# cvg/nice-slam

Hardware: NVIDIA H100
Metric: rendered rays/sec (higher is better)
Workload: dtype f32

## Files before the change

### nice_slam_b200/csrc/nsb_common.cuh

```cuda
#pragma once
#include <cuda_runtime.h>
#include <cuda_fp16.h>
#include <stdint.h>
#include "../../include/nice_slam_b200.h"

namespace nsb {

constexpr int kHid = 32;
constexpr int kEmb = 93;
constexpr int kEmbPad = 96;
constexpr int kChunk = 16;
constexpr int kRowF = 16;
constexpr int kMaxPtsPerBlock = 384;
constexpr int kMaxRaysPerBlock = 24;

__host__ __device__ inline size_t align16(size_t x) { return (x + 15) & ~size_t(15); }

template <int LV>
struct Dec {
  static constexpr bool XYZ = LV != 0;
  static constexpr int CD = LV == 2 ? 64 : 32;
  static constexpr int NO = LV == 3 ? 4 : 1;
  static constexpr int FIRST = XYZ ? kEmb : 32;
  static constexpr int FIRSTP = XYZ ? kEmbPad : 32;
// ... 129 lines not shown
  int max_n;
};
struct PeerTail { PeerX px; const double* loss; double* out13; };
struct FusedSeeds {
  int kind;
  const void* gt_rgb;
  const float* gt_depth_loss;
  double w_color;
  int handle_dynamic, use_color;
  double* g_depth; float* g_rgb; double* loss;
  double* res;
  int* counter;
  PeerX px;
};
int render_forward_fused(const nsb_render_inputs* in, const nsb_forward_outputs* out, const FusedSeeds* fs, void* stream,
                         const nsb_sampling* smp = nullptr);
int render_backward_tail(const nsb_render_inputs* in, const nsb_backward_args* bw, const PeerTail* tail, void* stream, bool after_forward = false,
                         const nsb_sampling* smp = nullptr);
int make_peerx(const struct nsb_peers* p, PeerX* px);
int eval_points_mesh(const nsb_render_inputs* in, const double* points, const nsb_mesh_lattice* lat, int n_points, float* raw, float* z,
                     void* stream);

size_t det_voxel_workspace_bytes(long long n_points);
int det_voxel_reduce(const nsb_grid& g, const int32_t* slot_map, const float* xn, const float* dc, long long n_points, float* d_grid,
                     void* workspace, size_t workspace_bytes, cudaStream_t st);
int det_tile_sum(const float* part, int tiles, int n_floats, float* out, cudaStream_t st);

void set_error(const char* fmt, ...);
int check_cuda(cudaError_t e, const char* what);

}
```

### nice_slam_b200/csrc/nsb_iter.cu

```cuda
#include <cstring>
#include "nsb_common.cuh"

using namespace nsb;

static size_t backward_offset(int n_rays) { return 16 + align16(nsb_tracking_seeds_workspace(n_rays)); }
static size_t split_offset(int n_rays) { return backward_offset(n_rays) + align16(nsb_backward_workspace_bytes()); }
extern "C" size_t nsb_iteration_workspace_bytes(int n_rays) {
  return split_offset(n_rays) + align16(nsb_split_workspace_bytes(n_rays, NSB_MAX_SAMPLES));
}
struct IterWs { int* seeds_counter; void* seeds_scratch; void* backward; void* split; size_t split_bytes; };
static IterWs carve(const nsb_iteration_buffers* b, int n_rays) {
  char* w = static_cast<char*>(b->workspace);
  return {reinterpret_cast<int*>(w), w + 16, w + backward_offset(n_rays), w + split_offset(n_rays), b->workspace_bytes - split_offset(n_rays)};
}

static int check_buffers(const nsb_render_inputs* in, const nsb_iteration_buffers* b, const nsb_backward_args* g) {
  if (!in || !b || !g) { set_error("iteration: NULL argument"); return NSB_ERR_ARG; }
  if (!b->depth || !b->var || !b->rgb || !b->z_vals || !b->raw || !b->g_depth || !b->g_rgb || !b->loss || !b->depth_max || !b->workspace) {
    set_error("iteration: incomplete nsb_iteration_buffers"); return NSB_ERR_ARG; }
  if (b->workspace_bytes < nsb_iteration_workspace_bytes(in->n_rays)) {
    int det = 0; nsb_get_option("deterministic", &det);
    set_error(det ? "iteration: workspace smaller than nsb_iteration_workspace_bytes(%d) with option deterministic on (size it after setting the option)"
                  : "iteration: workspace too small", in->n_rays);
    return NSB_ERR_ARG;
  }
  return NSB_OK;
}

static int forward_part(const nsb_render_inputs* in, const nsb_iteration_buffers* b, const IterWs& ws, nsb_render_inputs* in2, const FusedSeeds* fs,
                        void* stream, bool keep_depth_max = false) {
  *in2 = *in;
  if (!(keep_depth_max && in->depth_max != nullptr)) {
    in2->depth_max = nullptr;
    if (in->gt_depth && in->gt_depth_batch == nullptr && in->n_rays > NSB_INLINE_MAX_RAYS) {
      const int rc = nsb_batch_max_depth(in->gt_depth, in->n_rays, b->depth_max, stream); if (rc) return rc;
      in2->depth_max = b->depth_max;
    }
  }
  nsb_forward_outputs fo = {b->depth, b->var, b->rgb, b->z_vals, b->raw, nullptr, b->masks, ws.split, ws.split_bytes, b->acts, b->acts_levels};
  return render_forward_fused(in2, &fo, fs, stream);
}

static FusedSeeds fused_seeds(const nsb_iteration_buffers* b, const IterWs& ws, int kind, const void* gt_rgb, const float* gt_depth_loss, double w_color,
                              int handle_dynamic, int use_color, const PeerX* px) {
  FusedSeeds fs; memset(&fs, 0, sizeof(fs));
  fs.kind = kind; fs.gt_rgb = gt_rgb; fs.gt_depth_loss = gt_depth_loss; fs.w_color = w_color; fs.handle_dynamic = handle_dynamic; fs.use_color = use_color;
  fs.g_depth = b->g_depth; fs.g_rgb = b->g_rgb; fs.loss = b->loss; fs.counter = ws.seeds_counter;
  if (kind == 1) fs.res = static_cast<double*>(ws.seeds_scratch);
  if (px != nullptr) fs.px = *px;
  return fs;
}

static int backward_part(const nsb_render_inputs* in2, const nsb_iteration_buffers* b, const IterWs& ws, const nsb_backward_args* g, void* stream,
                         const PeerTail* tail = nullptr, bool after_forward = false) {
  nsb_backward_args bw = *g;
  bw.z_vals = b->z_vals; bw.raw = b->raw; bw.g_depth = b->g_depth; bw.g_var = nullptr; bw.g_rgb = b->g_rgb; bw.masks = b->masks; bw.acts = b->acts; bw.acts_levels = b->acts_levels;
  bw.workspace = ws.backward; bw.split_workspace = ws.split; bw.split_workspace_bytes = ws.split_bytes;
  if (b->event_bwd_begin) cudaEventRecord((cudaEvent_t)b->event_bwd_begin, (cudaStream_t)stream);
  const int rc = render_backward_tail(in2, &bw, tail, stream, after_forward && !b->event_bwd_begin);
  if (b->event_bwd_end) cudaEventRecord((cudaEvent_t)b->event_bwd_end, (cudaStream_t)stream);
  return rc;
}

extern "C" int nsb_tracking_iteration(const nsb_render_inputs* in, const nsb_iteration_buffers* buf, const double* gt_rgb,
                                      double w_color, int handle_dynamic, int use_color, const nsb_backward_args* grads, void* stream) {
  int rc = check_buffers(in, buf, grads); if (rc) return rc;
  if (!in->gt_depth) { set_error("tracking iteration needs gt_depth"); return NSB_ERR_ARG; }
  nsb_render_inputs in2;
  const bool fuse = in->n_rays > 0 && in->n_rays <= 512;
  if (fuse && use_color && !gt_rgb) { set_error("tracking iteration: use_color without gt_rgb"); return NSB_ERR_ARG; }
  const IterWs ws = carve(buf, in->n_rays);
  const FusedSeeds fs = fused_seeds(buf, ws, 1, gt_rgb, nullptr, w_color, handle_dynamic, use_color, nullptr);
  if ((rc = forward_part(in, buf, ws, &in2, fuse ? &fs : nullptr, stream))) return rc;
  if (!fuse && (rc = nsb_tracking_seeds(buf->depth, buf->var, buf->rgb, in->gt_depth, gt_rgb, in->n_rays, w_color, handle_dynamic, use_color,
// ... 39 lines not shown
```

### nice_slam_b200/csrc/nsb_render.cu

```cuda
#include <cstdarg>
#include <cstdio>
#include <cstring>
#include "nsb_common.cuh"
#include "nsb_geom.cuh"
#include "nsb_mlp.cuh"
#include "nsb_seeds.cuh"

namespace nsb {

__device__ __forceinline__ bool grid_fast(const nsb_grid& g) { return g.stride_c == 1; }

__device__ __forceinline__ float4 grid_load4(const nsb_grid& g, long long off, int c0, bool fast) {
  if (fast) return ldg_f4(g.data + off + c0);
  return make_float4(__ldg(g.data + off + (long long)c0 * g.stride_c), __ldg(g.data + off + (long long)(c0 + 1) * g.stride_c),
                     __ldg(g.data + off + (long long)(c0 + 2) * g.stride_c), __ldg(g.data + off + (long long)(c0 + 3) * g.stride_c));
}

__device__ __forceinline__ void gather_chunk(const nsb_grid& g, float* __restrict__ act, int row0, const float xn[3], int lane) {
  const bool fast = grid_fast(g);
  const int q = lane & 7;
#pragma unroll 2
  for (int it = 0; it < 4; it++) {
    const int pt = it * 4 + (lane >> 3);
    float x[3];
// ... 101 lines not shown
  int accumulate_rays;
  int split;
  int* group_done;
  float4* fwd_parts;
  double* ray_parts;
  int* ray_cnt;
  float4* tile_parts;
  int tile_rays;
  int kind_major;
  FusedSeeds fs;
  PeerTail tail;
  int acts_mask;
  int wbytes;
  int max_pts, max_rays;
  nsb_sampling smp;
};

struct MeshPoints { nsb_mesh_lattice lat; int lattice; float* z; };
struct DetParams { float* dc[4]; float* xn[4]; float* wpart[4]; };
__device__ __forceinline__ double lattice_value(const nsb_mesh_lattice& L, int a, int i) {
  return i == L.n[a] - 1 ? L.stop[a] : __dadd_rn(__dmul_rn((double)i, L.step[a]), L.start[a]);
}
__device__ __forceinline__ void mesh_point_geom(const KParams& P, const MeshPoints& M, long long gp, PointGeom& G) {
  double pin[3];
  if (M.lattice) {
    const long long nyz = (long long)M.lat.n[1] * M.lat.n[2];
    const int ix = (int)(gp / nyz), iy = (int)((gp - ix * nyz) / M.lat.n[2]), iz = (int)(gp - ix * nyz - (long long)iy * M.lat.n[2]);
    pin[0] = lattice_value(M.lat, 0, ix); pin[1] = lattice_value(M.lat, 1, iy); pin[2] = lattice_value(M.lat, 2, iz);
  } else {
    pin[0] = P.points[3 * gp]; pin[1] = P.points[3 * gp + 1]; pin[2] = P.points[3 * gp + 2];
// ... 137 lines not shown
  float carry = 1.0f;
  for (int base = 0; base < S; base += 32) {
    const int s = base + lane;
    const bool v = s < S;
    const float al = v ? sigmoid_f(10.0f * rw[4 * s + 3]) : 0.0f;
    const float q = v ? (1.0f - al) + 1e-10f : 1.0f;
    const float incl = warp_incl_prod(q, lane);
    float excl = __shfl_up_sync(0xffffffffu, incl, 1);
    if (lane == 0) excl = 1.0f;
    const float T = carry * excl;
    if (v) { wq[s] = al * T; if (tq) tq[s] = T; }
    carry *= __shfl_sync(0xffffffffu, incl, 31);
  }
}

__device__ __forceinline__ void composite_ray_outputs(const KParams& P, int ray, const float* rw, const double* z, float* wq, int lane) {
  const int S = P.S;
  ray_weights(rw, S, lane, wq, nullptr);
  __syncwarp();
  float c0 = 0.f, c1 = 0.f, c2 = 0.f; double dsum = 0.0;
  for (int s = lane; s < S; s += 32) {
    const float w = wq[s];
    c0 = fmaf(w, rw[4 * s], c0); c1 = fmaf(w, rw[4 * s + 1], c1); c2 = fmaf(w, rw[4 * s + 2], c2);
    dsum += (double)w * z[s];
  }
  c0 = warp_sum(c0); c1 = warp_sum(c1); c2 = warp_sum(c2); dsum = warp_sum(dsum);
  double v = 0.0;
  for (int s = lane; s < S; s += 32) { const double t = z[s] - dsum; v += (double)wq[s] * t * t; }
  v = warp_sum(v);
  if (lane == 0) {
    P.fo.depth[ray] = dsum; P.fo.var[ray] = v;
    P.fo.rgb[3 * ray] = c0; P.fo.rgb[3 * ray + 1] = c1; P.fo.rgb[3 * ray + 2] = c2;
  }
}

template <typename F>
__device__ __forceinline__ void composite_ray_backward(const float* rw, const double* z, int S, double gD, double gV, const float g3[3],
                                                       float* wq, float* tq, int lane, F&& store) {
  ray_weights(rw, S, lane, wq, tq);
  __syncwarp();
  double Dm = 0.0;
  for (int s = lane; s < S; s += 32) Dm += (double)wq[s] * z[s];
  Dm = warp_sum(Dm);
  double swt = 0.0;
  for (int s = lane; s < S; s += 32) swt += (double)wq[s] * (z[s] - Dm);
  swt = warp_sum(swt);
  const double gDe = gD + gV * (-2.0 * swt);
  float carry = 0.0f;
  const int nblk = (S + 31) / 32;
  for (int b = nblk - 1; b >= 0; b--) {
    const int s = b * 32 + lane;
    const bool v = s < S;
    float gw = 0.0f, al = 0.0f, T = 0.0f, w = 0.0f;
    if (v) {
      al = sigmoid_f(10.0f * rw[4 * s + 3]); T = tq[s]; w = wq[s];
      const double t = z[s] - Dm;
      gw = (float)(gDe * z[s] + gV * t * t) + g3[0] * rw[4 * s] + g3[1] * rw[4 * s + 1] + g3[2] * rw[4 * s + 2];
    }
    const float incl = warp_incl_suffix_sum(gw * w, lane);
    float excl = __shfl_down_sync(0xffffffffu, incl, 1);
    if (lane == 31) excl = 0.0f;
    const float R = carry + excl;
    if (v) {
      const float qd = (1.0f - al) + 1e-10f;
      store(s, w, al, T * gw - R / qd);
    }
    carry += __shfl_sync(0xffffffffu, incl, 0);
  }
}

__device__ __forceinline__ void store_ray_grad(const KParams& P, int ray, int a, double so, double sd) {
  if (P.accumulate_rays) {
    if (P.bw.d_rays_o != nullptr) so += (double)P.bw.d_rays_o[3 * ray + a];
    if (P.bw.d_rays_d != nullptr) sd += (double)P.bw.d_rays_d[3 * ray + a];
  }
  if (P.bw.d_rays_o != nullptr) P.bw.d_rays_o[3 * ray + a] = (float)so;
  if (P.bw.d_rays_d != nullptr) P.bw.d_rays_d[3 * ray + a] = (float)sd;
}

__device__ __forceinline__ void issue_weights(const KParams& P, const Smem& sm, int lv) {
  fence_proxy_async();
  const uint32_t bytes = (uint32_t)packed_floats(lv) * 4u;
  mbar_expect_tx(sm.bar, bytes);
// ... 76 lines not shown
}
__device__ __forceinline__ void fwd_composite_store(const KParams& P, const Smem& sm, const BlockRange& b, int warp, int warps, int lane) {
  const int r0 = b.r0, nr = b.nr, Pb = b.Pb;
  if (P.points != nullptr) {
    for (int lp = threadIdx.x; lp < Pb; lp += blockDim.x) {
      const long long gp = (long long)blockIdx.x * P.rays_per_block + lp;
      float4 v = *reinterpret_cast<float4*>(sm.raw + 4 * lp);
      if (!sm.inb[lp]) v.w = 100.0f;
      *reinterpret_cast<float4*>(P.points_raw + 4 * gp) = v;
    }
    return;
  }
  for (int lp = threadIdx.x; lp < Pb; lp += blockDim.x) if (!sm.inb[lp]) sm.raw[4 * lp + 3] = 100.0f;
  __syncthreads();
  for (int r = warp; r < nr; r += warps)
    composite_ray_outputs(P, r0 + r, sm.raw + 4 * r * P.S, sm.zs + r * P.S, sm.wgt + r * P.S, lane);
  const long long g0 = (long long)r0 * P.S;
  if (P.fo.z_vals != nullptr) for (int lp = threadIdx.x; lp < Pb; lp += blockDim.x) P.fo.z_vals[g0 + lp] = sm.zs[lp];
  if (P.fo.raw != nullptr)
    for (int lp = threadIdx.x; lp < Pb; lp += blockDim.x)
      *reinterpret_cast<float4*>(P.fo.raw + 4 * (g0 + lp)) = *reinterpret_cast<float4*>(sm.raw + 4 * lp);
}

__device__ __forceinline__ void fused_seeds_tail(const KParams& P, int n_participants, unsigned char* scratch) {
  if (P.fs.kind == 0) return;
  __shared__ int s_seeds_last;
  if (!grid_last_arrival(P.fs.counter, n_participants, &s_seeds_last)) return;
  if (P.fs.kind == 1) {
    tracking_seeds_body(P.fo.depth, P.fo.var, P.fo.rgb, P.in.gt_depth, static_cast<const double*>(P.fs.gt_rgb), P.in.n_rays, P.fs.w_color,
                        P.fs.handle_dynamic, P.fs.use_color, nullptr, 0, P.fs.g_depth, P.fs.g_rgb, P.fs.loss, P.fs.res, P.fs.px, scratch);
    if (P.fs.px.world > 1 && P.in.depth_max == nullptr && P.in.gt_depth_batch == nullptr && threadIdx.x == 0) peer_advance(P.fs.px, 0);
// ... 536 lines not shown
}

static void fill_common(KParams& K, const nsb_render_inputs* in) {
  K.in = *in;
  K.has_gt = (in->gt_depth != nullptr && in->stage != NSB_STAGE_COARSE) ? 1 : 0;
  K.S = in->n_samples + (K.has_gt ? in->n_surface : 0);
  K.n_dec = stage_decoders(in->stage, K.dec);
  for (int i = 0; i < 3; i++) K.dec_pos[i] = i;
  K.accumulate_rays = 0;
  K.split = 1; K.group_done = nullptr; K.fwd_parts = nullptr; K.ray_parts = nullptr; K.ray_cnt = nullptr; K.tile_parts = nullptr; K.tile_rays = 0; K.kind_major = 0;
  memset(&K.fs, 0, sizeof(K.fs)); memset(&K.tail, 0, sizeof(K.tail));
  K.points = nullptr; K.points_raw = nullptr; K.n_points = 0;
  K.acts_mask = in->stage == NSB_STAGE_COLOR ? 1 << NSB_COLOR : 0;
  memset(&K.smp, 0, sizeof(K.smp));
  for (int l = 0; l < 4; l++) K.d_packed[l] = nullptr;
}

constexpr int kMaxDevices = 64;
static int g_sm_count[kMaxDevices] = {0};
static int current_device() { int dev = 0; cudaGetDevice(&dev); return dev >= 0 && dev < kMaxDevices ? dev : 0; }
static int sm_count() {
  const int dev = current_device();
  if (g_sm_count[dev] == 0) { cudaDeviceGetAttribute(&g_sm_count[dev], cudaDevAttrMultiProcessorCount, dev); if (g_sm_count[dev] <= 0) g_sm_count[dev] = 132; }
  return g_sm_count[dev];
}

constexpr size_t kSmemCap = 226u * 1024u;
constexpr int kMaxPtsTc = 256;
static void choose_config(KParams& K, bool bwd, int max_pts_cap, int* warps = nullptr, size_t* smem = nullptr) {
  const int sms = sm_count();
// ... 260 lines not shown
  K.smp = *smp;
  if (smp->z_vals != nullptr) {
    if (smp->S < 1) { set_error("nsb_sampling.S = %d with a given z_vals", smp->S); return NSB_ERR_ARG; }
    K.S = smp->S; K.smp.lindisp = 0; K.smp.t_rand = nullptr;
  }
  return NSB_OK;
}

extern "C" int nsb_render_forward(const nsb_render_inputs* in, const nsb_forward_outputs* out, void* stream) {
  return nsb_render_forward_sampled(in, nullptr, out, stream);
}
extern "C" int nsb_render_forward_sampled(const nsb_render_inputs* in, const nsb_sampling* sampling, const nsb_forward_outputs* out, void* stream) {
  return nsb::render_forward_fused(in, out, nullptr, stream, sampling);
}
int nsb::render_forward_fused(const nsb_render_inputs* in, const nsb_forward_outputs* out, const nsb::FusedSeeds* fs, void* stream,
                              const nsb_sampling* smp) {
  int rc = validate_inputs(in, true); if (rc) return rc;
  if (!out || !out->depth || !out->var || !out->rgb) { set_error("forward outputs missing"); return NSB_ERR_ARG; }
  if (in->n_rays == 0) return NSB_OK;
  KParams K; fill_common(K, in); K.fo = *out; memset(&K.bw, 0, sizeof(K.bw));
  if ((rc = apply_sampling(K, smp))) return rc;
  if ((rc = apply_acts_levels(K, out->acts_levels))) return rc;
  if (fs != nullptr) K.fs = *fs;
  const Family fam = kernel_family(K.S, in->n_rays, false);
  if (fam == Family::Fma) K.fo.masks = nullptr;
  if (K.S > NSB_MAX_SAMPLES) { set_error("n_samples+n_surface = %d exceeds %d", K.S, NSB_MAX_SAMPLES); return NSB_ERR_UNSUPPORTED; }
  if (K.has_gt && in->n_surface > 0 && !in->t_surface) { set_error("t_surface NULL"); return NSB_ERR_ARG; }
  if ((rc = set_attrs())) return rc;
  if (K.fs.px.world > 1 && !(fam != Family::Fma && in->gt_depth != nullptr)) {
    set_error("in-kernel exchanges of a sharded forward need a tensor-core back-end and <= %d rays per rank", NSB_INLINE_MAX_RAYS); return NSB_ERR_UNSUPPORTED; }
  if (fam == Family::Tile) {
    if (!out->z_vals || !out->raw) { set_error("the tensor-core forward needs z_vals and raw outputs"); return NSB_ERR_ARG; }
    if ((rc = plan_tile_ws(K, split_layout(in->n_rays, K.S, false), out->split_workspace, out->split_workspace_bytes, false, 2))) return rc;
    return launch_tile_fwd(K, (long long)in->n_rays * K.S, (cudaStream_t)stream);
  }
  if (fam == Family::Group) return launch_group(K, false, out->split_workspace, out->split_workspace_bytes, (cudaStream_t)stream);
  return launch_fma(K, false, (cudaStream_t)stream);
}

int nsb::eval_points_mesh(const nsb_render_inputs* in, const double* points, const nsb_mesh_lattice* lat, int n_points, float* raw, float* z,
                          void* stream) {
  int rc = validate_inputs(in, false); if (rc) return rc;
  if (n_points == 0) return NSB_OK;
  if (kernel_family(1, 0, true) != Family::Tile) { set_error("mesh extraction runs on the tile kernels (mlp_backend 0 or 3)"); return NSB_ERR_UNSUPPORTED; }
  KParams K; fill_common(K, in); memset(&K.fo, 0, sizeof(K.fo)); memset(&K.bw, 0, sizeof(K.bw));
  K.points = points; K.points_raw = raw; K.n_points = n_points; K.S = 1; K.has_gt = 0;
  MeshPoints M; memset(&M, 0, sizeof(M));
  if (lat != nullptr) { M.lat = *lat; M.lattice = 1; M.z = z; }
// ... 17 lines not shown

namespace nsb { int launch_unpack_grads(float* const d_packed[4], float* const d_flat[4], cudaStream_t st); }

static size_t backward_ws_offset(int l) {
  size_t o = 0; for (int m = 0; m < l; m++) o += align16((size_t)packed_floats(m) * 4); return o;
}
extern "C" size_t nsb_backward_workspace_bytes(void) { return backward_ws_offset(4); }

extern "C" int nsb_render_backward(const nsb_render_inputs* in, const nsb_backward_args* bw, void* stream) {
  return nsb_render_backward_sampled(in, nullptr, bw, stream);
}
extern "C" int nsb_render_backward_sampled(const nsb_render_inputs* in, const nsb_sampling* sampling, const nsb_backward_args* bw, void* stream) {
  return nsb::render_backward_tail(in, bw, nullptr, stream, false, sampling);
}
int nsb::render_backward_tail(const nsb_render_inputs* in, const nsb_backward_args* bw, const nsb::PeerTail* tail, void* stream, bool after_forward,
                              const nsb_sampling* smp) {
  int rc = validate_inputs(in, true); if (rc) return rc;
  if (!bw || !bw->z_vals || !bw->raw) { set_error("backward needs z_vals and raw from the forward pass"); return NSB_ERR_ARG; }
  if (in->n_rays == 0) return NSB_OK;
  KParams K; fill_common(K, in); K.bw = *bw; memset(&K.fo, 0, sizeof(K.fo));
  if ((rc = apply_sampling(K, smp))) return rc;
  if ((rc = apply_acts_levels(K, bw->acts_levels))) return rc;
  if (K.S > NSB_MAX_SAMPLES) { set_error("n_samples+n_surface = %d exceeds %d", K.S, NSB_MAX_SAMPLES); return NSB_ERR_UNSUPPORTED; }
  cudaStream_t st = (cudaStream_t)stream;
  bool any_w = false;
  const bool want_pose = bw->pose_dirs != nullptr;
  if (want_pose && (!bw->d_c2w || !bw->pose_counter || !bw->d_rays_o || !bw->d_rays_d)) {
    set_error("pose_dirs given without d_c2w / pose_counter / d_rays_o / d_rays_d"); return NSB_ERR_ARG; }
  if (bw->result_dst != nullptr) {
    if (!want_pose) { set_error("result_dst needs pose_dirs (the block is stored by the CTA that produces d c2w)"); return NSB_ERR_ARG; }
    if (tail != nullptr && tail->px.world > 1) { set_error("result_dst is not supported by the sharded backward tail"); return NSB_ERR_ARG; }
// ... 68 lines not shown
      const int lv = K.dec[j];
      bool in_launch = false; for (int q = 0; q < P.n_dec; q++) in_launch |= P.dec[q] == lv;
      if (!in_launch) continue;
      if (P.bw.d_grid[lv] != nullptr) { D.dc[lv] = dw.dc[j]; D.xn[lv] = dw.xn[j]; }
      if (wg) D.wpart[lv] = dw.wpart[lv > 0 ? lv - 1 : 0];
    }
    return D;
  };
  for (int i = 0; i < n; i++) {
    KParams& P = L[i];
    const bool wg = kind[i] == WgTile;
    if (kind[i] == GroupIg) rc = launch_group(P, true, bw->split_workspace, bw->split_workspace_bytes, st);
    else if (kind[i] == Fma) rc = launch_fma(P, true, st);
    else if (!(rc = plan_tile_ws(P, W, bw->split_workspace, bw->split_workspace_bytes, true, wg ? 1 : 2))) {
      const DetParams D = det_params(P, wg);
      rc = launch_tile_bwd(P, wg, det ? &D : nullptr, after_forward && !any_w && g_pdl, st);
    }
    if (rc) return rc;
  }
  for (int j = 0; j < K.n_dec && det; j++) {
    const int lv = K.dec[j];
    if (K.bw.d_grid[lv] != nullptr &&
        (rc = det_voxel_reduce(in->grid[lv], bw->slot_map[lv], dw.xn[j], dw.dc[j], NP, K.bw.d_grid[lv], dw.sort, dw.sort_bytes, st))) return rc;
  }
  if (any_w && (rc = launch_unpack_grads(K.d_packed, bw->d_flat, st))) return rc;
  if (kind[n - 1] == Fma && want_pose) {
    if ((rc = nsb_pose_grad(bw->pose_dirs, bw->d_rays_o, bw->d_rays_d, in->n_rays, bw->d_c2w, stream))) return rc;
    if (bw->result_dst != nullptr) return nsb_copy_block(bw->result_dst, bw->result_src, bw->result_bytes, stream);
  }
  return NSB_OK;
// ... 43 lines not shown
```

### nice_slam_b200/csrc/nsb_tile.cuh

```cuda
#pragma once

namespace nsb {
namespace tl {

using tc::TM;
constexpr int kThreads = 256;
constexpr int kEpiThreads = kThreads;
constexpr int kCG = 2, kCW = 16, kKQ = 4;
constexpr int kSlots = 4;
constexpr int kSlotFloatsFwd = 2560;
constexpr int kSlotFloatsBwd = 2048;
constexpr int kABufFloats = 2 * TM * 32;
constexpr int kMaxTileRays = 18;
constexpr int kMinSamples = 8;
constexpr long long kWaitCycles = 4000000000ll;

enum { B_FULL = 0, B_EMPTY = 4, B_HDR = 8, B_AREADY = 10, B_DONE = 12, kNumBars = 14 };

__device__ __forceinline__ bool mbar_try(uint64_t* bar, uint32_t parity) {
  uint32_t ok;
  asm volatile("{\n\t.reg .pred p;\n\tmbarrier.try_wait.parity.shared::cta.b64 p, [%1], %2;\n\tselp.b32 %0, 1, 0, p;\n\t}"
               : "=r"(ok) : "r"(smem_u32(bar)), "r"(parity) : "memory");
  return ok != 0;
}
// ... 605 lines not shown
  for (int j = 0; j < 2; j++) { const float give = (lane & 8) ? b[j] : b[j + 2], keep = (lane & 8) ? b[j + 2] : b[j]; c[j] = keep + __shfl_xor_sync(0xffffffffu, give, 8); }
  const float give = (lane & 4) ? c[0] : c[1], keep = (lane & 4) ? c[1] : c[0];
  return keep + __shfl_xor_sync(0xffffffffu, give, 4);
}
__device__ __forceinline__ int frag_colsum_col(int lane) {
  const int j = ((lane >> 4) & 1) * 4 + ((lane >> 3) & 1) * 2 + ((lane >> 2) & 1);
  return 8 * (j >> 1) + 2 * (lane & 3) + (j & 1);
}

struct BwdExtra {
  double dp[TM * 3];
  double z[TM];
  float gocc[TM];
  float wgt[TM];
  float gc[kMaxTileRays * 3];
};
__device__ __forceinline__ void bwd_gout(const BwdExtra& X, int lv, int r, int npts, int off0, int S, float (&go)[4]) {
  go[0] = go[1] = go[2] = go[3] = 0.0f;
  if (r >= npts) return;
  if (lv == 3) { const float w = X.wgt[r]; const float* gc = X.gc + 3 * ((off0 + r) / S); go[0] = w * gc[0]; go[1] = w * gc[1]; go[2] = w * gc[2]; }
  else go[0] = X.gocc[r];
}

template <bool DC, int NDF, bool L0>
__device__ __forceinline__ void issue_bwd_layer_t(Issuer& I, const TileSmem& t, int ndc, float (&d1)[16], float (&dc)[16], float (&fa)[16]) {
  constexpr int ND1 = L0 ? 0 : 1, FMAX = L0 ? 2 : 1;
  constexpr int kWaves = NDF > FMAX ? (NDF + FMAX - 1) / FMAX : 1;
#pragma unroll
  for (int wave = 0; wave < kWaves; wave++) {
    const int f0 = wave * FMAX;
// ... 329 lines not shown
  __threadfence();
  if (threadIdx.x == 0) *s_ndone = 0;
  __syncthreads();
  if ((int)threadIdx.x < nr) {
    const int ray = ray_lo + threadIdx.x;
    const int target = tiles_of_ray(ray, S) * per_tile;
    const int old = atomicAdd(ray_cnt + ray, 1);
    if (old == target - 1) { ray_cnt[ray] = 0; s_done[atomicAdd(s_ndone, 1)] = ray; }
  }
  __syncthreads();
  const int nd = *s_ndone;
  if (nd > 0) __threadfence();
  return nd;
}

__host__ __device__ inline size_t composite_scratch_bytes(int S) { return ((size_t)28 * S + 15) & ~size_t(15); }
__device__ __forceinline__ void composite_ray(const KParams& P, int ray, int lane, unsigned char* scratch) {
  const int S = P.S;
  float* rw = reinterpret_cast<float*>(scratch);
  double* zz = reinterpret_cast<double*>(rw + 4 * S);
  float* wq = reinterpret_cast<float*>(zz + S);
  float o[3], d[3];
#pragma unroll
  for (int a = 0; a < 3; a++) { o[a] = P.in.rays_o[3 * ray + a]; d[a] = P.in.rays_d[3 * ray + a]; }
  const long long g0 = (long long)ray * S, NS = (long long)P.in.n_rays * S;
  for (int s = lane; s < S; s += 32) {
    float4 pq[3];
#pragma unroll
    for (int q = 0; q < 3; q++) pq[q] = q < P.split ? __ldcg(P.tile_parts + q * NS + g0 + s) : make_float4(0.f, 0.f, 0.f, 0.f);
    const double z = __ldcg(P.fo.z_vals + g0 + s);
    float4 v = make_float4(0.f, 0.f, 0.f, 0.f);
#pragma unroll
    for (int q = 0; q < 3; q++) { v.x += pq[q].x; v.y += pq[q].y; v.z += pq[q].z; v.w += pq[q].w; }
    PointGeom G; make_point(P.in.bound, P.in.coarse_bound, o, d, z, G);
    if (!G.inb) v.w = 100.0f;
    zz[s] = z;
    *reinterpret_cast<float4*>(rw + 4 * s) = v;
    *reinterpret_cast<float4*>(P.fo.raw + 4 * (g0 + s)) = v;
  }
  __syncwarp();
  composite_ray_outputs(P, ray, rw, zz, wq, lane);
  __syncwarp();
}

}

template <bool H16, bool kSampled = false, bool kMesh = false>
__device__ __forceinline__ void render_fwd_tile_body(const KParams& P, const MeshPoints* M = nullptr) {
  extern __shared__ __align__(1024) unsigned char smem_raw[];
  using namespace tl;
  const int tid = threadIdx.x, warp = tid >> 5, lane = tid & 31;
  const int row = tid & (TM - 1), cg = tid >> 7;
  TileSmem t; carve(smem_raw, t, false);
  __shared__ int s_ndone, s_done[kMaxTileRays];
  __shared__ float s_max[16];
  __shared__ uint32_t s_seq;

// ... 85 lines not shown
  if (threadIdx.x == 0) tc::acc_release(acc_slot);
  asm volatile("griddepcontrol.launch_dependents;" ::: "memory");
  NSB_PH(14);
  NSB_ITEM_MARK(0, 1, P, item);

  if (points) {
    if (cg == 0 && row < npts) {
      if (kMesh && M->z != nullptr) M->z[gp0 + row] = G.inb ? occ : 100.0f;
      else *reinterpret_cast<float4*>(P.points_raw + 4 * (gp0 + row)) = make_float4(c0, c1, c2, G.inb ? occ : 100.0f);
    }
    return;
  }
  if (cg == 0 && row < npts) P.tile_parts[(long long)my * NP + gp0 + row] = make_float4(c0, c1, c2, occ);
  const int nd = complete_rays(P.ray_cnt, ray_lo, nr, S, nsplit, s_done, &s_ndone);
  NSB_PH(15);
  for (int k = warp; k < nd; k += kThreads / 32) composite_ray(P, s_done[k], lane, smem_raw + (size_t)warp * composite_scratch_bytes(S));
  NSB_PH(16);
  fused_seeds_tail(P, gridDim.x, smem_raw);
  NSB_ITEM_MARK(0, 2, P, item);
}
__global__ void __launch_bounds__(tl::kThreads, 2) render_fwd_tile_kernel(const __grid_constant__ KParams P) { render_fwd_tile_body<false>(P); }
__global__ void __launch_bounds__(tl::kThreads, 2) render_fwd_tile_h16_kernel(const __grid_constant__ KParams P) { render_fwd_tile_body<true>(P); }
__global__ void __launch_bounds__(tl::kThreads, 2) render_fwd_tile_sampled_kernel(const __grid_constant__ KParams P) { render_fwd_tile_body<false, true>(P); }
__global__ void __launch_bounds__(tl::kThreads, 2) render_fwd_tile_mesh_kernel(const __grid_constant__ KParams P, const __grid_constant__ MeshPoints M) {
  render_fwd_tile_body<false, false, true>(P, &M);
}

template <int WG, bool kDet = false>
__device__ __forceinline__ void render_bwd_tile_body(const KParams& P, const DetParams* D = nullptr) {
  extern __shared__ __align__(1024) unsigned char smem_raw[];
  using namespace tl;
// ... 17 lines not shown
  const long long gp0 = (long long)tile * TM;
  const int npts = (int)(NP - gp0 < TM ? NP - gp0 : TM);
  const int ray_lo = (int)(gp0 / S), nr = (int)((gp0 + npts - 1) / S) - ray_lo + 1;

  if (threadIdx.x == 0) *t.tmem = tc::acc_acquire();
  NSB_PH_RESET();
  Issuer I; I.L.P = &P; I.L.q = q0; I.L.q1 = q1; I.L.k = 0; I.L.loaded = 0; I.L.mode = 1; I.issued = 0; I.g = 0;
  if (tid == 0) {
    for (int i = 0; i < kNumBars; i++) mbar_init(t.bars + i, (i >= B_EMPTY && i < B_EMPTY + kSlots) ? 2 : 1);
    mbar_fence_init();
    load_header(P, t, P.dec[q0], 0);
    for (int i = 0; i < kSlots; i++) loader_issue(I.L, t);
  }

  for (int i = tid; i < TM * 3; i += kThreads) X.dp[i] = 0.0;
  asm volatile("griddepcontrol.wait;" ::: "memory");
  for (int r = warp; r < nr; r += kThreads / 32) {
    const int ray = ray_lo + r;
    float* rw = t.a[0] + (size_t)warp * ((6 * S + 3) & ~3);
    float* wq = rw + 4 * S; float* go = wq + S;
    const long long g0 = (long long)ray * S;
    float o[3], d[3];
#pragma unroll
    for (int a = 0; a < 3; a++) { o[a] = P.in.rays_o[3 * ray + a]; d[a] = P.in.rays_d[3 * ray + a]; }
    for (int s = lane; s < S; s += 32) *reinterpret_cast<float4*>(rw + 4 * s) = *reinterpret_cast<const float4*>(P.bw.raw + 4 * (g0 + s));
    __syncwarp();
    float g3[3] = {0.f, 0.f, 0.f};
    if (P.bw.g_rgb != nullptr) { g3[0] = P.bw.g_rgb[3 * ray]; g3[1] = P.bw.g_rgb[3 * ray + 1]; g3[2] = P.bw.g_rgb[3 * ray + 2]; }
    if (lane == 0) { X.gc[3 * r] = g3[0]; X.gc[3 * r + 1] = g3[1]; X.gc[3 * r + 2] = g3[2]; }
    const double* z = P.bw.z_vals + g0;
    composite_ray_backward(rw, z, S, P.bw.g_depth != nullptr ? P.bw.g_depth[ray] : 0.0, P.bw.g_var != nullptr ? P.bw.g_var[ray] : 0.0, g3,
                           wq, go, lane, [&](int s, float w, float al, float ga) {
      const long long gp = g0 + s;
      if (gp >= gp0 && gp < gp0 + npts) {
        PointGeom Gs; make_point(P.in.bound, P.in.coarse_bound, o, d, z[s], Gs);
        X.gocc[gp - gp0] = Gs.inb ? 10.0f * al * (1.0f - al) * ga : 0.0f;
        X.wgt[gp - gp0] = w;
      }
    });
  }
  NSB_PH(20);
  PointGeom G;
  const int lp = row < npts ? row : npts - 1;
  const long long gpr = gp0 + lp;
  const int rayr = (int)(gpr / S);
  {
    float o[3], d[3];
#pragma unroll
    for (int a = 0; a < 3; a++) { o[a] = P.in.rays_o[3 * rayr + a]; d[a] = P.in.rays_d[3 * rayr + a]; }
    const double z = P.bw.z_vals[gpr];
    make_point(P.in.bound, P.in.coarse_bound, o, d, z, G);
    if (cg == 0) X.z[row] = z;
  }
  __syncthreads();
  const uint32_t acc_slot = *t.tmem;
  NSB_PH(21);

  {
    const int off0 = (int)(gp0 - (long long)ray_lo * S);
    for (int qd = q0; qd < q1; qd++) {
      const int lv = P.dec[qd];
      const uint32_t* gm = P.bw.masks + (gp0 * 15 + P.dec_pos[qd] * 5);
      const int dq = qd - q0;
      if (tid == 0 && qd + 1 < q1) load_header(P, t, P.dec[qd + 1], (dq + 1) & 1);
      if constexpr (kDet) { if (WG) wg.dpk = D->wpart[lv] + (size_t)tile * packed_floats(lv); }
      else if (WG) wg.dpk = P.d_packed[lv];
      const float* acts_row = (WG && row < npts) ? P.bw.acts + ((acts_slot(P.acts_mask, lv) * NP + gp0 + row) * 5) * 32 + kCW * cg : nullptr;
      epi_backward<WG, kDet>(P, t, I, X, lv, G, dq & 1, (dq >> 1) & 1u, gm, npts, off0, gp0, WG ? &wg : nullptr, acts_row);
      epi_sync();
// ... 70 lines not shown
```

Before: 1.324 million.

## Precompute per-point compositing gradient coefficients in forward to skip backward ray scans

While compositing each ray, the forward tile kernel now computes per-point coefficients: the sigmoid-derivative factor times the suffix-scan terms for depth and each RGB channel, plus the weight. It writes them to a new workspace buffer. The backward tile kernel then builds the occupancy gradient as a small dot product of these coefficients with the per-ray upstream gradients, replacing the per-ray backward scan over raw and z_vals. This linearity holds only when there is no variance gradient, so that case falls back to the old path. The cost is extra forward work, 32 bytes per point of global memory traffic, and a larger workspace.

Measured after the change: 1.327 million (median of 6 runs). Within noise of the previous version (+0.2%).

```diff
diff --git a/nice_slam_b200/csrc/nsb_common.cuh b/nice_slam_b200/csrc/nsb_common.cuh
--- a/nice_slam_b200/csrc/nsb_common.cuh
+++ b/nice_slam_b200/csrc/nsb_common.cuh
@@ -167,9 +167,10 @@
   PeerX px;
 };
 int render_forward_fused(const nsb_render_inputs* in, const nsb_forward_outputs* out, const FusedSeeds* fs, void* stream,
-                         const nsb_sampling* smp = nullptr);
+                         const nsb_sampling* smp = nullptr, float* coef = nullptr);
 int render_backward_tail(const nsb_render_inputs* in, const nsb_backward_args* bw, const PeerTail* tail, void* stream, bool after_forward = false,
-                         const nsb_sampling* smp = nullptr);
+                         const nsb_sampling* smp = nullptr, const float* coef = nullptr);
+inline size_t render_coef_bytes(long long n_points) { return (size_t)n_points * 8 * sizeof(float); }
 int make_peerx(const struct nsb_peers* p, PeerX* px);
 int eval_points_mesh(const nsb_render_inputs* in, const double* points, const nsb_mesh_lattice* lat, int n_points, float* raw, float* z,
                      void* stream);
diff --git a/nice_slam_b200/csrc/nsb_iter.cu b/nice_slam_b200/csrc/nsb_iter.cu
--- a/nice_slam_b200/csrc/nsb_iter.cu
+++ b/nice_slam_b200/csrc/nsb_iter.cu
@@ -4,14 +4,16 @@
 using namespace nsb;
 
 static size_t backward_offset(int n_rays) { return 16 + align16(nsb_tracking_seeds_workspace(n_rays)); }
-static size_t split_offset(int n_rays) { return backward_offset(n_rays) + align16(nsb_backward_workspace_bytes()); }
+static size_t coef_offset(int n_rays) { return backward_offset(n_rays) + align16(nsb_backward_workspace_bytes()); }
+static size_t split_offset(int n_rays) { return coef_offset(n_rays) + align16(render_coef_bytes((long long)n_rays * NSB_MAX_SAMPLES)); }
 extern "C" size_t nsb_iteration_workspace_bytes(int n_rays) {
   return split_offset(n_rays) + align16(nsb_split_workspace_bytes(n_rays, NSB_MAX_SAMPLES));
 }
-struct IterWs { int* seeds_counter; void* seeds_scratch; void* backward; void* split; size_t split_bytes; };
+struct IterWs { int* seeds_counter; void* seeds_scratch; void* backward; float* coef; void* split; size_t split_bytes; };
 static IterWs carve(const nsb_iteration_buffers* b, int n_rays) {
   char* w = static_cast<char*>(b->workspace);
-  return {reinterpret_cast<int*>(w), w + 16, w + backward_offset(n_rays), w + split_offset(n_rays), b->workspace_bytes - split_offset(n_rays)};
+  return {reinterpret_cast<int*>(w), w + 16, w + backward_offset(n_rays), reinterpret_cast<float*>(w + coef_offset(n_rays)), w + split_offset(n_rays),
+          b->workspace_bytes - split_offset(n_rays)};
 }
 
 static int check_buffers(const nsb_render_inputs* in, const nsb_iteration_buffers* b, const nsb_backward_args* g) {
@@ -38,7 +40,7 @@
     }
   }
   nsb_forward_outputs fo = {b->depth, b->var, b->rgb, b->z_vals, b->raw, nullptr, b->masks, ws.split, ws.split_bytes, b->acts, b->acts_levels};
-  return render_forward_fused(in2, &fo, fs, stream);
+  return render_forward_fused(in2, &fo, fs, stream, nullptr, ws.coef);
 }
 
 static FusedSeeds fused_seeds(const nsb_iteration_buffers* b, const IterWs& ws, int kind, const void* gt_rgb, const float* gt_depth_loss, double w_color,
@@ -57,7 +59,7 @@
   bw.z_vals = b->z_vals; bw.raw = b->raw; bw.g_depth = b->g_depth; bw.g_var = nullptr; bw.g_rgb = b->g_rgb; bw.masks = b->masks; bw.acts = b->acts; bw.acts_levels = b->acts_levels;
   bw.workspace = ws.backward; bw.split_workspace = ws.split; bw.split_workspace_bytes = ws.split_bytes;
   if (b->event_bwd_begin) cudaEventRecord((cudaEvent_t)b->event_bwd_begin, (cudaStream_t)stream);
-  const int rc = render_backward_tail(in2, &bw, tail, stream, after_forward && !b->event_bwd_begin);
+  const int rc = render_backward_tail(in2, &bw, tail, stream, after_forward && !b->event_bwd_begin, nullptr, ws.coef);
   if (b->event_bwd_end) cudaEventRecord((cudaEvent_t)b->event_bwd_end, (cudaStream_t)stream);
   return rc;
 }
diff --git a/nice_slam_b200/csrc/nsb_render.cu b/nice_slam_b200/csrc/nsb_render.cu
--- a/nice_slam_b200/csrc/nsb_render.cu
+++ b/nice_slam_b200/csrc/nsb_render.cu
@@ -139,6 +139,7 @@
   int wbytes;
   int max_pts, max_rays;
   nsb_sampling smp;
+  float* coef;
 };
 
 struct MeshPoints { nsb_mesh_lattice lat; int lattice; float* z; };
@@ -306,9 +307,9 @@
   }
 }
 
-__device__ __forceinline__ void composite_ray_outputs(const KParams& P, int ray, const float* rw, const double* z, float* wq, int lane) {
+__device__ __forceinline__ void composite_ray_outputs(const KParams& P, int ray, const float* rw, const double* z, float* wq, float* tq, int lane) {
   const int S = P.S;
-  ray_weights(rw, S, lane, wq, nullptr);
+  ray_weights(rw, S, lane, wq, tq);
   __syncwarp();
   float c0 = 0.f, c1 = 0.f, c2 = 0.f; double dsum = 0.0;
   for (int s = lane; s < S; s += 32) {
@@ -323,6 +324,33 @@
   if (lane == 0) {
     P.fo.depth[ray] = dsum; P.fo.var[ray] = v;
     P.fo.rgb[3 * ray] = c0; P.fo.rgb[3 * ray + 1] = c1; P.fo.rgb[3 * ray + 2] = c2;
+  }
+}
+
+template <int NC, typename CW, typename F>
+__device__ __forceinline__ void alpha_grad_scan(const float* rw, const float* wq, const float* tq, int S, int lane, CW&& cw, F&& store) {
+  float carry[NC];
+#pragma unroll
+  for (int j = 0; j < NC; j++) carry[j] = 0.0f;
+  const int nblk = (S + 31) / 32;
+  for (int b = nblk - 1; b >= 0; b--) {
+    const int s = b * 32 + lane;
+    const bool v = s < S;
+    float c[NC], al = 0.0f, T = 0.0f, w = 0.0f;
+#pragma unroll
+    for (int j = 0; j < NC; j++) c[j] = 0.0f;
+    if (v) { al = sigmoid_f(10.0f * rw[4 * s + 3]); T = tq[s]; w = wq[s]; cw(s, c); }
+    const float qd = (1.0f - al) + 1e-10f;
+    float K[NC];
+#pragma unroll
+    for (int j = 0; j < NC; j++) {
+      const float incl = warp_incl_suffix_sum(c[j] * w, lane);
+      float excl = __shfl_down_sync(0xffffffffu, incl, 1);
+      if (lane == 31) excl = 0.0f;
+      K[j] = T * c[j] - (carry[j] + excl) / qd;
+      carry[j] += __shfl_sync(0xffffffffu, incl, 0);
+    }
+    if (v) store(s, w, al, K);
   }
 }
 
@@ -338,27 +366,25 @@
   for (int s = lane; s < S; s += 32) swt += (double)wq[s] * (z[s] - Dm);
   swt = warp_sum(swt);
   const double gDe = gD + gV * (-2.0 * swt);
-  float carry = 0.0f;
-  const int nblk = (S + 31) / 32;
-  for (int b = nblk - 1; b >= 0; b--) {
-    const int s = b * 32 + lane;
-    const bool v = s < S;
-    float gw = 0.0f, al = 0.0f, T = 0.0f, w = 0.0f;
-    if (v) {
-      al = sigmoid_f(10.0f * rw[4 * s + 3]); T = tq[s]; w = wq[s];
-      const double t = z[s] - Dm;
-      gw = (float)(gDe * z[s] + gV * t * t) + g3[0] * rw[4 * s] + g3[1] * rw[4 * s + 1] + g3[2] * rw[4 * s + 2];
-    }
-    const float incl = warp_incl_suffix_sum(gw * w, lane);
-    float excl = __shfl_down_sync(0xffffffffu, incl, 1);
-    if (lane == 31) excl = 0.0f;
-    const float R = carry + excl;
-    if (v) {
-      const float qd = (1.0f - al) + 1e-10f;
-      store(s, w, al, T * gw - R / qd);
-    }
-    carry += __shfl_sync(0xffffffffu, incl, 0);
-  }
+  alpha_grad_scan<1>(rw, wq, tq, S, lane, [&](int s, float (&c)[1]) {
+    const double t = z[s] - Dm;
+    c[0] = (float)(gDe * z[s] + gV * t * t) + g3[0] * rw[4 * s] + g3[1] * rw[4 * s + 1] + g3[2] * rw[4 * s + 2];
+  }, [&](int s, float w, float al, const float (&K)[1]) { store(s, w, al, K[0]); });
+}
+
+template <int J0, int NJ>
+__device__ __forceinline__ void composite_ray_coefs(float* coef, const float* rw, const double* z, const float* wq, const float* tq, const float* fq,
+                                                    int S, int lane) {
+  static_assert(J0 % 2 == 0 && NJ % 2 == 0 && J0 + NJ <= 4, "components are stored in pairs");
+  alpha_grad_scan<NJ>(rw, wq, tq, S, lane, [&](int s, float (&c)[NJ]) {
+#pragma unroll
+    for (int j = 0; j < NJ; j++) c[j] = J0 + j == 0 ? (float)z[s] : rw[4 * s + J0 + j - 1];
+  }, [&](int s, float w, float, const float (&K)[NJ]) {
+    const float f = fq[s];
+#pragma unroll
+    for (int j = 0; j < NJ; j += 2) __stcg(reinterpret_cast<float2*>(coef + 8 * s + J0 + j), make_float2(f * K[j], f * K[j + 1]));
+    if (J0 == 0) __stcg(coef + 8 * s + 4, w);
+  });
 }
 
 __device__ __forceinline__ void store_ray_grad(const KParams& P, int ray, int a, double so, double sd) {
@@ -465,7 +491,7 @@
   for (int lp = threadIdx.x; lp < Pb; lp += blockDim.x) if (!sm.inb[lp]) sm.raw[4 * lp + 3] = 100.0f;
   __syncthreads();
   for (int r = warp; r < nr; r += warps)
-    composite_ray_outputs(P, r0 + r, sm.raw + 4 * r * P.S, sm.zs + r * P.S, sm.wgt + r * P.S, lane);
+    composite_ray_outputs(P, r0 + r, sm.raw + 4 * r * P.S, sm.zs + r * P.S, sm.wgt + r * P.S, nullptr, lane);
   const long long g0 = (long long)r0 * P.S;
   if (P.fo.z_vals != nullptr) for (int lp = threadIdx.x; lp < Pb; lp += blockDim.x) P.fo.z_vals[g0 + lp] = sm.zs[lp];
   if (P.fo.raw != nullptr)
@@ -1032,6 +1058,7 @@
   K.acts_mask = in->stage == NSB_STAGE_COLOR ? 1 << NSB_COLOR : 0;
   memset(&K.smp, 0, sizeof(K.smp));
   for (int l = 0; l < 4; l++) K.d_packed[l] = nullptr;
+  K.coef = nullptr;
 }
 
 constexpr int kMaxDevices = 64;
@@ -1322,7 +1349,7 @@
   return nsb::render_forward_fused(in, out, nullptr, stream, sampling);
 }
 int nsb::render_forward_fused(const nsb_render_inputs* in, const nsb_forward_outputs* out, const nsb::FusedSeeds* fs, void* stream,
-                              const nsb_sampling* smp) {
+                              const nsb_sampling* smp, float* coef) {
   int rc = validate_inputs(in, true); if (rc) return rc;
   if (!out || !out->depth || !out->var || !out->rgb) { set_error("forward outputs missing"); return NSB_ERR_ARG; }
   if (in->n_rays == 0) return NSB_OK;
@@ -1340,6 +1367,7 @@
   if (fam == Family::Tile) {
     if (!out->z_vals || !out->raw) { set_error("the tensor-core forward needs z_vals and raw outputs"); return NSB_ERR_ARG; }
     if ((rc = plan_tile_ws(K, split_layout(in->n_rays, K.S, false), out->split_workspace, out->split_workspace_bytes, false, 2))) return rc;
+    K.coef = coef;
     return launch_tile_fwd(K, (long long)in->n_rays * K.S, (cudaStream_t)stream);
   }
   if (fam == Family::Group) return launch_group(K, false, out->split_workspace, out->split_workspace_bytes, (cudaStream_t)stream);
@@ -1387,7 +1415,7 @@
   return nsb::render_backward_tail(in, bw, nullptr, stream, false, sampling);
 }
 int nsb::render_backward_tail(const nsb_render_inputs* in, const nsb_backward_args* bw, const nsb::PeerTail* tail, void* stream, bool after_forward,
-                              const nsb_sampling* smp) {
+                              const nsb_sampling* smp, const float* coef) {
   int rc = validate_inputs(in, true); if (rc) return rc;
   if (!bw || !bw->z_vals || !bw->raw) { set_error("backward needs z_vals and raw from the forward pass"); return NSB_ERR_ARG; }
   if (in->n_rays == 0) return NSB_OK;
@@ -1486,6 +1514,7 @@
     else if (kind[i] == Fma) rc = launch_fma(P, true, st);
     else if (!(rc = plan_tile_ws(P, W, bw->split_workspace, bw->split_workspace_bytes, true, wg ? 1 : 2))) {
       const DetParams D = det_params(P, wg);
+      P.coef = bw->g_var == nullptr ? const_cast<float*>(coef) : nullptr;
       rc = launch_tile_bwd(P, wg, det ? &D : nullptr, after_forward && !any_w && g_pdl, st);
     }
     if (rc) return rc;
diff --git a/nice_slam_b200/csrc/nsb_tile.cuh b/nice_slam_b200/csrc/nsb_tile.cuh
--- a/nice_slam_b200/csrc/nsb_tile.cuh
+++ b/nice_slam_b200/csrc/nsb_tile.cuh
@@ -643,6 +643,7 @@
   float gocc[TM];
   float wgt[TM];
   float gc[kMaxTileRays * 3];
+  float gd[kMaxTileRays];
 };
 __device__ __forceinline__ void bwd_gout(const BwdExtra& X, int lv, int r, int npts, int off0, int S, float (&go)[4]) {
   go[0] = go[1] = go[2] = go[3] = 0.0f;
@@ -1002,12 +1003,16 @@
   return nd;
 }
 
-__host__ __device__ inline size_t composite_scratch_bytes(int S) { return ((size_t)28 * S + 15) & ~size_t(15); }
-__device__ __forceinline__ void composite_ray(const KParams& P, int ray, int lane, unsigned char* scratch) {
+__host__ __device__ inline size_t composite_scratch_bytes(int S) { return ((size_t)36 * S + 15) & ~size_t(15); }
+struct CompositeScratch {
+  float* rw; double* zz; float* wq; float* tq; float* fq;
+  __device__ CompositeScratch(unsigned char* p, int S) {
+    rw = reinterpret_cast<float*>(p); zz = reinterpret_cast<double*>(rw + 4 * S); wq = reinterpret_cast<float*>(zz + S); tq = wq + S; fq = tq + S;
+  }
+};
+__device__ __forceinline__ void composite_ray(const KParams& P, int ray, int lane, unsigned char* scratch, bool coefs) {
   const int S = P.S;
-  float* rw = reinterpret_cast<float*>(scratch);
-  double* zz = reinterpret_cast<double*>(rw + 4 * S);
-  float* wq = reinterpret_cast<float*>(zz + S);
+  const CompositeScratch C(scratch, S);
   float o[3], d[3];
 #pragma unroll
   for (int a = 0; a < 3; a++) { o[a] = P.in.rays_o[3 * ray + a]; d[a] = P.in.rays_d[3 * ray + a]; }
@@ -1022,13 +1027,20 @@
     for (int q = 0; q < 3; q++) { v.x += pq[q].x; v.y += pq[q].y; v.z += pq[q].z; v.w += pq[q].w; }
     PointGeom G; make_point(P.in.bound, P.in.coarse_bound, o, d, z, G);
     if (!G.inb) v.w = 100.0f;
-    zz[s] = z;
-    *reinterpret_cast<float4*>(rw + 4 * s) = v;
+    if (P.coef != nullptr) { const float al = sigmoid_f(10.0f * v.w); C.fq[s] = G.inb ? 10.0f * al * (1.0f - al) : 0.0f; }
+    C.zz[s] = z;
+    *reinterpret_cast<float4*>(C.rw + 4 * s) = v;
     *reinterpret_cast<float4*>(P.fo.raw + 4 * (g0 + s)) = v;
   }
   __syncwarp();
-  composite_ray_outputs(P, ray, rw, zz, wq, lane);
+  composite_ray_outputs(P, ray, C.rw, C.zz, C.wq, P.coef != nullptr ? C.tq : nullptr, lane);
+  if (coefs) composite_ray_coefs<0, 4>(P.coef + 8 * g0, C.rw, C.zz, C.wq, C.tq, C.fq, S, lane);
   __syncwarp();
+}
+template <int J0>
+__device__ __forceinline__ void composite_ray_coefs_of(const KParams& P, int ray, int lane, unsigned char* scratch) {
+  const CompositeScratch C(scratch, P.S);
+  composite_ray_coefs<J0, 2>(P.coef + 8 * (long long)ray * P.S, C.rw, C.zz, C.wq, C.tq, C.fq, P.S, lane);
 }
 
 }
@@ -1144,7 +1156,15 @@
   if (cg == 0 && row < npts) P.tile_parts[(long long)my * NP + gp0 + row] = make_float4(c0, c1, c2, occ);
   const int nd = complete_rays(P.ray_cnt, ray_lo, nr, S, nsplit, s_done, &s_ndone);
   NSB_PH(15);
-  for (int k = warp; k < nd; k += kThreads / 32) composite_ray(P, s_done[k], lane, smem_raw + (size_t)warp * composite_scratch_bytes(S));
+  const bool pair_coefs = P.coef != nullptr && nd <= kThreads / 64;
+  for (int k = warp; k < nd; k += kThreads / 32)
+    composite_ray(P, s_done[k], lane, smem_raw + (size_t)warp * composite_scratch_bytes(S), P.coef != nullptr && !pair_coefs);
+  if (pair_coefs) {
+    __syncthreads();
+    const int k = warp % (kThreads / 64);
+    unsigned char* sc = smem_raw + (size_t)k * composite_scratch_bytes(S);
+    if (k < nd) { if (warp < kThreads / 64) composite_ray_coefs_of<0>(P, s_done[k], lane, sc); else composite_ray_coefs_of<2>(P, s_done[k], lane, sc); }
+  }
   NSB_PH(16);
   fused_seeds_tail(P, gridDim.x, smem_raw);
   NSB_ITEM_MARK(0, 2, P, item);
@@ -1192,45 +1212,65 @@
   }
 
   for (int i = tid; i < TM * 3; i += kThreads) X.dp[i] = 0.0;
-  asm volatile("griddepcontrol.wait;" ::: "memory");
-  for (int r = warp; r < nr; r += kThreads / 32) {
-    const int ray = ray_lo + r;
-    float* rw = t.a[0] + (size_t)warp * ((6 * S + 3) & ~3);
-    float* wq = rw + 4 * S; float* go = wq + S;
-    const long long g0 = (long long)ray * S;
-    float o[3], d[3];
-#pragma unroll
-    for (int a = 0; a < 3; a++) { o[a] = P.in.rays_o[3 * ray + a]; d[a] = P.in.rays_d[3 * ray + a]; }
-    for (int s = lane; s < S; s += 32) *reinterpret_cast<float4*>(rw + 4 * s) = *reinterpret_cast<const float4*>(P.bw.raw + 4 * (g0 + s));
-    __syncwarp();
-    float g3[3] = {0.f, 0.f, 0.f};
-    if (P.bw.g_rgb != nullptr) { g3[0] = P.bw.g_rgb[3 * ray]; g3[1] = P.bw.g_rgb[3 * ray + 1]; g3[2] = P.bw.g_rgb[3 * ray + 2]; }
-    if (lane == 0) { X.gc[3 * r] = g3[0]; X.gc[3 * r + 1] = g3[1]; X.gc[3 * r + 2] = g3[2]; }
-    const double* z = P.bw.z_vals + g0;
-    composite_ray_backward(rw, z, S, P.bw.g_depth != nullptr ? P.bw.g_depth[ray] : 0.0, P.bw.g_var != nullptr ? P.bw.g_var[ray] : 0.0, g3,
-                           wq, go, lane, [&](int s, float w, float al, float ga) {
-      const long long gp = g0 + s;
-      if (gp >= gp0 && gp < gp0 + npts) {
-        PointGeom Gs; make_point(P.in.bound, P.in.coarse_bound, o, d, z[s], Gs);
-        X.gocc[gp - gp0] = Gs.inb ? 10.0f * al * (1.0f - al) * ga : 0.0f;
-        X.wgt[gp - gp0] = w;
-      }
-    });
-  }
-  NSB_PH(20);
-  PointGeom G;
   const int lp = row < npts ? row : npts - 1;
   const long long gpr = gp0 + lp;
   const int rayr = (int)(gpr / S);
+  float o[3], d[3];
+#pragma unroll
+  for (int a = 0; a < 3; a++) { o[a] = P.in.rays_o[3 * rayr + a]; d[a] = P.in.rays_d[3 * rayr + a]; }
+  asm volatile("griddepcontrol.wait;" ::: "memory");
+  PointGeom G;
+  float4 cf0; float cf1;
+  if (P.coef != nullptr) {
+    if (cg == 0) { const float4* c = reinterpret_cast<const float4*>(P.coef + 8 * gpr); cf0 = __ldcg(c); cf1 = __ldcg(P.coef + 8 * gpr + 4); }
+    if (tid < nr) {
+      const int ray = ray_lo + tid;
+      X.gd[tid] = P.bw.g_depth != nullptr ? (float)P.bw.g_depth[ray] : 0.0f;
+#pragma unroll
+      for (int c = 0; c < 3; c++) X.gc[3 * tid + c] = P.bw.g_rgb != nullptr ? P.bw.g_rgb[3 * ray + c] : 0.0f;
+    }
+  } else {
+    for (int r = warp; r < nr; r += kThreads / 32) {
+      const int ray = ray_lo + r;
+      float* rw = t.a[0] + (size_t)warp * ((6 * S + 3) & ~3);
+      float* wq = rw + 4 * S; float* go = wq + S;
+      const long long g0 = (long long)ray * S;
+      float ro[3], rd[3];
+#pragma unroll
+      for (int a = 0; a < 3; a++) { ro[a] = P.in.rays_o[3 * ray + a]; rd[a] = P.in.rays_d[3 * ray + a]; }
+      for (int s = lane; s < S; s += 32) *reinterpret_cast<float4*>(rw + 4 * s) = *reinterpret_cast<const float4*>(P.bw.raw + 4 * (g0 + s));
+      __syncwarp();
+      float g3[3] = {0.f, 0.f, 0.f};
+      if (P.bw.g_rgb != nullptr) { g3[0] = P.bw.g_rgb[3 * ray]; g3[1] = P.bw.g_rgb[3 * ray + 1]; g3[2] = P.bw.g_rgb[3 * ray + 2]; }
+      if (lane == 0) { X.gc[3 * r] = g3[0]; X.gc[3 * r + 1] = g3[1]; X.gc[3 * r + 2] = g3[2]; }
+      const double* z = P.bw.z_vals + g0;
+      composite_ray_backward(rw, z, S, P.bw.g_depth != nullptr ? P.bw.g_depth[ray] : 0.0, P.bw.g_var != nullptr ? P.bw.g_var[ray] : 0.0, g3,
+                             wq, go, lane, [&](int s, float w, float al, float ga) {
+        const long long gp = g0 + s;
+        if (gp >= gp0 && gp < gp0 + npts) {
+          PointGeom Gs; make_point(P.in.bound, P.in.coarse_bound, ro, rd, z[s], Gs);
+          X.gocc[gp - gp0] = Gs.inb ? 10.0f * al * (1.0f - al) * ga : 0.0f;
+          X.wgt[gp - gp0] = w;
+        }
+      });
+    }
+  }
+  NSB_PH(20);
   {
-    float o[3], d[3];
-#pragma unroll
-    for (int a = 0; a < 3; a++) { o[a] = P.in.rays_o[3 * rayr + a]; d[a] = P.in.rays_d[3 * rayr + a]; }
     const double z = P.bw.z_vals[gpr];
     make_point(P.in.bound, P.in.coarse_bound, o, d, z, G);
     if (cg == 0) X.z[row] = z;
   }
   __syncthreads();
+  if (P.coef != nullptr) {
+    if (cg == 0 && row < npts) {
+      const int r = rayr - ray_lo;
+      const float* g3 = X.gc + 3 * r;
+      X.gocc[row] = fmaf(X.gd[r], cf0.x, fmaf(g3[0], cf0.y, fmaf(g3[1], cf0.z, g3[2] * cf0.w)));
+      X.wgt[row] = cf1;
+    }
+    __syncthreads();
+  }
   const uint32_t acc_slot = *t.tmem;
   NSB_PH(21);
 
```
